# chenchen235/SemStereo

Measured on AMD Instinct MI355X. Metric: stereo pairs/sec, hot segment (gwc+concat volumes, 3-D hourglass stack, soft-argmax), 1024x1024 maxdisp=128, higher is better.
Workload: dtype f32; 1 GPU; BASELINE.json configs[1]: 1024x1024, maxdisp=128, batch=1/GPU x 1 GPU(s); features [B,128,H/4,W/4]+[B,256,H/8,W/8] -> disparity; input_sets_rotated=3, execution=steps round-robin on 6 HIP streams (PairPipeline); bit-identical to one stream, conv_engine=f16x3, hip_graph=False

## Files before the change

include/semstereo_hip.h:

```cpp
#ifndef SEMSTEREO_HIP_H
#define SEMSTEREO_HIP_H

#ifdef __cplusplus
extern "C" {
#endif

typedef void* ss_stream_t;

enum ss_status {
    SS_OK = 0,
    SS_ERR_INVALID = -1,
    SS_ERR_UNSUPPORTED = -2,
    SS_ERR_LAUNCH = -3
};

int ss_abi_version(void);
int ss_reload_tuning(void);
const char* ss_status_string(int status);
const char* ss_last_hip_error(void);


int ss_groupwise_correlation_fwd(const float* fea1, const float* fea2, float* out,
                                 int B, int C, int H, int W, int groups, int normalize,
                                 ss_stream_t stream);
// ... 120 lines not shown
int ss_conv3d_bf16s_cl_fwd(const float* in, const void* wsplit, const float* scale, const float* shift, float* out,
                           int B, int Cin, int D, int H, int W, int Cout, int relu, int nterms, ss_stream_t stream);
int ss_conv3d_head_bf16s_cl_fwd(const float* in, const void* wsplit, const float* scale, const float* shift,
                                float* out, int B, int Cin, int D, int H, int W, int relu, int nterms,
                                ss_stream_t stream);
int ss_pack_classifier_head_weights(const float* w2, void* out, ss_stream_t stream);
int ss_conv3d_classifier_fused_fwd(const float* in, const void* wsplit, const float* scale, const float* shift,
                                   const void* head_w, float* patches, float* out, int B, int Cin, int D, int H, int W,
                                   int nterms, ss_stream_t stream);
int ss_regression_topk_patched_fwd(const float* patches, const float* samples, float* out, int B, int nd, int H, int W, int k,
                                   ss_stream_t stream);
int ss_conv3d_pointwise_bf16s_fwd(const float* in, const void* wsplit, const float* scale, const float* shift,
                                  float* out, int B, int Cin, int Cout, long long npos, int relu, int nterms,
                                  ss_stream_t stream);
int ss_pack_pointwise_weights_bf16s(const float* w, void* wsplit, int Cout, int Cin, ss_stream_t stream);

int ss_deconv3d_fwd(const float* in, const float* wpack, const float* scale, const float* shift,
                    const float* skip, const float* skip_wpack, const float* skip_scale, const float* skip_shift,
                    float* out, int B, int Cin, int D, int H, int W, int Cout, int Cs, int relu,
                    ss_stream_t stream);
int ss_deconv3d_bf16s_fwd(const float* in, const void* wsplit, const float* shift, const float* skip,
                          const void* skip_wsplit, float* out, int B, int Cin, int D, int H, int W, int Cout,
                          int Cs, int relu, int nterms, ss_stream_t stream);
int ss_pack_deconv3d_weights_bf16s(const float* wpack, void* wsplit, int Cin, int Cout, int ntaps, ss_stream_t stream);
int ss_pack_deconv3d_weights_f16s(const float* wpack, void* wsplit, int Cin, int Cout, ss_stream_t stream);
int ss_pack_conv3d_weights(const float* w, float* wpack, int Cout, int Cin, int k, int transposed,
                           ss_stream_t stream);
int ss_conv3d_wgrad_fwd(const float* grad_out, const float* in, float* grad_w, int B, int Cin, int D, int H, int W,
                        int Cout, int stride, ss_stream_t stream);
int ss_conv3d_wgrad_bf16s_fwd(const float* grad_out, const float* in, float* grad_w, float* workspace, int B, int Cin, int D, int H,
// ... 94 lines not shown
```

semstereo_amd/_lib.py:

```python
import ctypes
import os

import torch

_HERE = os.path.dirname(os.path.abspath(__file__))
LIB_PATH = os.path.join(_HERE, "csrc", "libsemstereo_hip.so")
ABI_VERSION = 20

_P = ctypes.c_void_p
_I = ctypes.c_int

_SIGNATURES = {
    "ss_groupwise_correlation_fwd": [_P, _P, _P, _I, _I, _I, _I, _I, _I, _P],
    "ss_gwc_volume_fwd": [_P, _P, _P, _I, _I, _I, _I, _I, _I, _I, _I, _P],
    "ss_gwc_patch_gate_fwd": [_P, _P, _P, _P, _P, _I, _I, _I, _I, _I, _I, _I, _I, _P],
    "ss_gwc_volume_bwd": [_P, _P, _P, _P, _P, _I, _I, _I, _I, _I, _I, _I, _P],
    "ss_concat_volume_fwd": [_P, _P, _P, _I, _I, _I, _I, _I, _I, _I, _P],
    "ss_concat_volume_bwd": [_P, _P, _P, _I, _I, _I, _I, _I, _I, _I, _P],
    "ss_warp_sampled_fwd": [_P, _P, _P, _P, _P, _I, _I, _I, _I, _I, _P],
    "ss_warp_sampled_bwd": [_P, _P, _P, _P, _P, _P, _P, _I, _I, _I, _I, _I, _P],
    "ss_concat_sampled_fwd": [_P, _P, _P, _P, _P, _I, _I, _I, _I, _I, _P],
    "ss_concat_sampled_bwd": [_P, _P, _P, _P, _P, _P, _P, _P, _I, _I, _I, _I, _I, _I, _P],
    "ss_concat_sampled_presplit_fwd": [_P, _P, _P, _P, _P, _I, _I, _I, _I, _I, _P],
    "ss_conv3d_presplit_fwd": [_P, _P, _P, _P, _P, _P, _P, _P, _I, _I, _I, _I, _I, _I, _I, _P],
# ... 27 lines not shown
    "ss_conv2d_bf16s_cat_fwd": [_P, _P, _P, _P, _P, _P, _P, _P, _I, _I, _I, _I, _I, _I, _I, _I, _P],
    "ss_deconv2d_bf16s_fwd": [_P, _P, _P, _P, _P, _I, _I, _I, _I, _I, _I, _I, _P],
    "ss_deconv2d_bf16s_pair_fwd": [_P, _P, _P, _P, _P, _P, _I, _I, _I, _I, _I, _I, _I, _P],
    "ss_pack_deconv2d_weights_f16s": [_P, _P, _I, _I, _P],
    "ss_pack_conv2d_weights_f16s": [_P, _P, _I, _I, _P],
    "ss_conv3d_head_bf16s_fwd": [_P, _P, _P, _P, _P, _I, _I, _I, _I, _I, _I, _I, _P],
    "ss_conv3d_head_bf16s_cl_fwd": [_P, _P, _P, _P, _P, _I, _I, _I, _I, _I, _I, _I, _P],
    "ss_conv3d_bf16s_cl_fwd": [_P, _P, _P, _P, _P, _I, _I, _I, _I, _I, _I, _I, _I, _P],
    "ss_pack_classifier_head_weights": [_P, _P, _P],
    "ss_conv3d_classifier_fused_fwd": [_P, _P, _P, _P, _P, _P, _P, _I, _I, _I, _I, _I, _I, _P],
    "ss_regression_topk_patched_fwd": [_P, _P, _P, _I, _I, _I, _I, _I, _P],
    "ss_pack_conv3d_head_weights_bf16s": [_P, _P, _I, _P],
    "ss_pack_conv3d_head_weights_f16s": [_P, _P, _I, _P],
    "ss_conv3d_pointwise_bf16s_fwd": [_P, _P, _P, _P, _P, _I, _I, _I, ctypes.c_longlong, _I, _I, _P],
    "ss_pack_pointwise_weights_bf16s": [_P, _P, _I, _I, _P],
    "ss_deconv3d_fwd": [_P, _P, _P, _P, _P, _P, _P, _P, _P, _I, _I, _I, _I, _I, _I, _I, _I, _P],
    "ss_pack_deconv3d_weights_f16s": [_P, _P, _I, _I, _P],
    "ss_deconv3d_bf16s_fwd": [_P, _P, _P, _P, _P, _P, _I, _I, _I, _I, _I, _I, _I, _I, _I, _P],
    "ss_pack_deconv3d_weights_bf16s": [_P, _P, _I, _I, _I, _P],
    "ss_pack_conv3d_weights": [_P, _P, _I, _I, _I, _I, _P],
    "ss_conv3d_wgrad_fwd": [_P, _P, _P, _I, _I, _I, _I, _I, _I, _I, _P],
    "ss_conv3d_wgrad_bf16s_fwd": [_P, _P, _P, _P, _I, _I, _I, _I, _I, _I, _I, _P],
    "ss_depthwise_patch_fwd": [_P, _P, _P, _P, _I, _I, _I, _I, _I, _P],
    "ss_window_attention_fwd": [_P, _P, _P, _P, _P, _P, _I, _I, _I, _I, _I, _I, _I, _I, _I, _P],
    "ss_window_attention_core_fwd": [_P, _P, _P, _I, _I, _I, _I, _I, _I, _I, _I, _I, _P],
    "ss_tool_copy_fwd": [_P, _P, ctypes.c_longlong, _P],
    "ss_upsample_softmax_regression_bwd": [_P, _P, _P, _P, _P, _P, _I, _I, _I, _I, _I, _P],
    "ss_sample_strength_bwd": [_P, _P, _P, _P, _P, _P, _P, _P, _P, _P, _P, _P, _I, _I, _I, _I, _P],
    "ss_sample_strength_bwd_ws": [_P, _P, _P, _P, _P, _P, _P, _P, _P, _P, _P, _P, _P, _I, _I, _I, _I, _P],
    "ss_topk_candidates_bwd": [_P, _P, _P, _P, _P, _P, _P, _I, _I, _I, _I, _I, _I, _P],
# ... 94 lines not shown
```

semstereo_amd/csrc/conv3d_head.hip:

```cpp
#include <algorithm>

#include "common.h"
#include "split_f16.h"

namespace {

using f32x16 = __attribute__((ext_vector_type(16))) float;
using bf16x8 = __attribute__((ext_vector_type(8))) short;
using bf16x2_t = __attribute__((ext_vector_type(2))) __bf16;
using f32x2_t = __attribute__((ext_vector_type(2))) float;

constexpr int TWO = 30;

__device__ __forceinline__ unsigned cvt_pk_bf16(float x0, float x1) {
    const f32x2_t v = {x0, x1};
    return __builtin_bit_cast(unsigned, __builtin_convertvector(v, bf16x2_t));
}
__device__ __forceinline__ void split3_pk(float x0, float x1, unsigned& h, unsigned& m, unsigned& l) {
    h = cvt_pk_bf16(x0, x1);
    const float r0 = x0 - __uint_as_float(h << 16), r1 = x1 - __uint_as_float(h & 0xffff0000u);
    m = cvt_pk_bf16(r0, r1);
    const float s0 = r0 - __uint_as_float(m << 16), s1 = r1 - __uint_as_float(m & 0xffff0000u);
    l = cvt_pk_bf16(s0, s1);
}
// ... 244 lines not shown
                           : launch_head_tile<KSV, F16X3>(in, wsplit, scale, shift, out, B, D, H, W, relu, st);
    SS_HEAD(1)
    SS_HEAD(2)
    SS_HEAD(4)
#undef SS_HEAD
    return SS_ERR_UNSUPPORTED;
}

namespace {

template <int KS, int NTERMS>
__global__ __launch_bounds__(256, 2) void pointwise_bf16s(const float* __restrict__ in, const uint4* __restrict__ wsplit,
                                                           const float* __restrict__ scale, const float* __restrict__ shift,
                                                           float* __restrict__ out, int Cout, long long npos,
                                                           int tiles_per_wave, int relu) {
    constexpr int NC = (NTERMS == 6) ? 3 : 2;
    constexpr int Cin = KS * 16;
    const int tid = threadIdx.x, lane = tid & 63, wave = tid >> 6;
    const int l31 = lane & 31, half = lane >> 5;
    const int mt = blockIdx.y * 4 + wave;
    const int b = blockIdx.z;
    if (mt * 32 >= Cout) return;
    bf16x8 a[KS][NC];
#pragma unroll
    for (int ks = 0; ks < KS; ++ks)
#pragma unroll
        for (int c = 0; c < NC; ++c)
            a[ks][c] = __builtin_bit_cast(bf16x8, wsplit[(((size_t)mt * KS + ks) * 3 + c) * 64 + half * 32 + l31]);

    const __amdgpu_buffer_rsrc_t ires = __builtin_amdgcn_make_buffer_rsrc(
        const_cast<float*>(in + (size_t)b * Cin * npos), 0, (int)min((long long)Cin * npos * 4, 0x7fffffffLL), 0x00020000);
    const int chan_b = (int)(npos * 4);
    const __amdgpu_buffer_rsrc_t ores = __builtin_amdgcn_make_buffer_rsrc(
        out + (size_t)b * Cout * npos, 0, (int)min((long long)Cout * npos * 4, 0x7fffffffLL), 0x00020000);
    __shared__ float aff[4][64];
    if (lane < 32) {
        const int co = min(mt * 32 + lane, Cout - 1);
        aff[wave][lane] = scale ? scale[co] : 1.0f;
        aff[wave][32 + lane] = shift ? shift[co] : 0.0f;
    }
    const float floor_v = relu ? 0.f : -__builtin_inff();
    const long long t0 = (long long)blockIdx.x * tiles_per_wave;
    float x[KS][8];
    auto lane_offset = [&](long long tile) {
        const long long p = tile * 32 + l31;
        return (p < npos) ? (unsigned)((8LL * half * npos + p) * 4) : 0x80000000u;
    };
    auto load_step = [&](unsigned off, int ks) {
#pragma unroll
        for (int j = 0; j < 8; ++j)
            x[ks][j] = __builtin_bit_cast(float, __builtin_amdgcn_raw_buffer_load_b32(ires, (int)off, (ks * 16 + j) * chan_b, 0));
    };
    {
        const unsigned off0 = lane_offset(t0);
#pragma unroll
        for (int ks = 0; ks < KS; ++ks) load_step(off0, ks);
    }
#pragma unroll 1
    for (int it = 0; it < tiles_per_wave; ++it) {
        const long long tile = t0 + it;
        if (tile * 32 >= npos) break;
        const unsigned offn = (it + 1 < tiles_per_wave) ? lane_offset(tile + 1) : 0x80000000u;
        f32x16 acc;
#pragma unroll
        for (int q = 0; q < 16; ++q) acc[q] = 0.f;
#pragma unroll
        for (int ks = 0; ks < KS; ++ks) {
            unsigned bh[4], bm[4], bl[4];
#pragma unroll
            for (int j = 0; j < 4; ++j) split3_pk(x[ks][2 * j], x[ks][2 * j + 1], bh[j], bm[j], bl[j]);
            load_step(offn, ks);
            const bf16x8 h8 = __builtin_bit_cast(bf16x8, make_uint4(bh[0], bh[1], bh[2], bh[3]));
            const bf16x8 m8 = __builtin_bit_cast(bf16x8, make_uint4(bm[0], bm[1], bm[2], bm[3]));
            if (NTERMS == 6) {
                const bf16x8 l8 = __builtin_bit_cast(bf16x8, make_uint4(bl[0], bl[1], bl[2], bl[3]));
                acc = __builtin_amdgcn_mfma_f32_32x32x16_bf16(a[ks][1], m8, acc, 0, 0, 0);
                acc = __builtin_amdgcn_mfma_f32_32x32x16_bf16(a[ks][0], l8, acc, 0, 0, 0);
                acc = __builtin_amdgcn_mfma_f32_32x32x16_bf16(a[ks][NC - 1], h8, acc, 0, 0, 0);
            }
            acc = __builtin_amdgcn_mfma_f32_32x32x16_bf16(a[ks][0], m8, acc, 0, 0, 0);
            acc = __builtin_amdgcn_mfma_f32_32x32x16_bf16(a[ks][1], h8, acc, 0, 0, 0);
            acc = __builtin_amdgcn_mfma_f32_32x32x16_bf16(a[ks][0], h8, acc, 0, 0, 0);
        }
        const long long p = tile * 32 + l31;
        const unsigned vo = (p < npos) ? (unsigned)((4LL * half * npos + p) * 4) : 0x80000000u;
#pragma unroll
        for (int r = 0; r < 16; ++r) {
            const int cl = (r & 3) + 8 * (r >> 2);
            const float v = fmaxf(ss::add_rn(ss::mul_rn(acc[r], aff[wave][cl + 4 * half]), aff[wave][32 + cl + 4 * half]), floor_v);
            __builtin_amdgcn_raw_buffer_store_b32(__builtin_bit_cast(unsigned, v), ores,
                                                  (int)((mt * 32 + cl + 4 * half < Cout) ? vo : 0x80000000u), (mt * 32 + cl) * chan_b, 0);
        }
    }
}

__global__ void pack_pointwise_weights_kernel(const float* __restrict__ w, unsigned short* __restrict__ wsplit, int Cout,
                                              int Cin, int total) {
    const int i = blockIdx.x * blockDim.x + threadIdx.x;
    if (i >= total) return;
    const int j = i % 8;
    int r = i / 8;
    const int row = r % 32; r /= 32;
    const int hk = r % 2; r /= 2;
    const int term = r % 3; r /= 3;
    const int KS = Cin / 16;
    const int ks = r % KS;
    const int mt = r / KS;
    const int co = mt * 32 + row, c = ks * 16 + 8 * hk + j;
    const float x = (co < Cout) ? w[(size_t)co * Cin + c] : 0.f;
    unsigned h, m, l;
    split3_pk(x, 0.f, h, m, l);
    wsplit[i] = (unsigned short)((term == 0 ? h : (term == 1 ? m : l)) & 0xffffu);
}

template <int KS, int NTERMS>
int launch_pointwise(const float* in, const void* wsplit, const float* scale, const float* shift, float* out, int B,
                     int Cout, long long npos, int relu, hipStream_t st) {
    const long long ntiles = (npos + 31) / 32;
    const int mgroups = ss::ceil_div(ss::ceil_div(Cout, 32), 4);
    int tpw = 8;
    while (tpw > 1 && ((ntiles + tpw - 1) / tpw) * mgroups * B < 1024) tpw >>= 1;
    const long long gx = (ntiles + tpw - 1) / tpw;
    if (gx > 0x7fffffffLL || B > 65535 || mgroups > 65535) return SS_ERR_UNSUPPORTED;
    hipLaunchKernelGGL((pointwise_bf16s<KS, NTERMS>), dim3((unsigned)gx, mgroups, B), dim3(256), 0, st, in,
                       reinterpret_cast<const uint4*>(wsplit), scale, shift, out, Cout, npos, tpw, relu);
    return ss::check_launch();
}

}

extern "C" int ss_pack_pointwise_weights_bf16s(const float* w, void* wsplit, int Cout, int Cin, ss_stream_t stream) {
    SS_REQUIRE(w && wsplit && Cout > 0 && Cin > 0 && Cin % 16 == 0);
    const int total = ss::ceil_div(Cout, 32) * (Cin / 16) * 3 * 2 * 32 * 8;
    hipLaunchKernelGGL(pack_pointwise_weights_kernel, dim3(ss::ceil_div(total, 256)), dim3(256), 0, ss::as_stream(stream), w,
                       reinterpret_cast<unsigned short*>(wsplit), Cout, Cin, total);
    return ss::check_launch();
}

extern "C" int ss_conv3d_pointwise_bf16s_fwd(const float* in, const void* wsplit, const float* scale, const float* shift,
                                             float* out, int B, int Cin, int Cout, long long npos, int relu, int nterms,
                                             ss_stream_t stream) {
    SS_REQUIRE(in && wsplit && out);
    SS_REQUIRE(B > 0 && Cin > 0 && Cout > 0 && npos > 0 && (nterms == 3 || nterms == 6));
    SS_REQUIRE((reinterpret_cast<uintptr_t>(wsplit) & 15) == 0);
    if ((long long)Cin * npos * 4 >= 0x7fffffffLL) return SS_ERR_UNSUPPORTED;
    if ((long long)Cout * npos * 4 >= 0x7fffffffLL) return SS_ERR_UNSUPPORTED;
    hipStream_t st = ss::as_stream(stream);
#define SS_PW(KSV)                                                                                                    \
    if (Cin == 16 * KSV)                                                                                              \
        return nterms == 6 ? launch_pointwise<KSV, 6>(in, wsplit, scale, shift, out, B, Cout, npos, relu, st)         \
                           : launch_pointwise<KSV, 3>(in, wsplit, scale, shift, out, B, Cout, npos, relu, st);
    SS_PW(2)
    SS_PW(4)
    SS_PW(8)
#undef SS_PW
    return SS_ERR_UNSUPPORTED;
}

extern "C" int ss_conv3d_head_bf16s_cl_fwd(const float* in, const void* wsplit, const float* scale, const float* shift,
                                           float* out, int B, int Cin, int D, int H, int W, int relu, int nterms,
                                           ss_stream_t stream) {
    SS_REQUIRE(in && wsplit && out);
    SS_REQUIRE(B > 0 && Cin > 0 && D > 0 && H > 0 && W > 0 && (nterms == 3 || nterms == 6 || nterms == F16X3));
    SS_REQUIRE(((reinterpret_cast<uintptr_t>(wsplit) | reinterpret_cast<uintptr_t>(in)) & 15) == 0);
    if ((long long)Cin * D * H * W * 4 >= 0x7fffffffLL) return SS_ERR_UNSUPPORTED;
    hipStream_t st = ss::as_stream(stream);
// ... 7 lines not shown
```

semstereo_amd/csrc/stem_left.hip:

```cpp
#include <algorithm>

#include "common.h"

namespace {

constexpr int TH = 8, TW = 32, COG = 4;

template <int ND>
__global__ __launch_bounds__(256) void stem_left_kernel(const float* __restrict__ q, const float* __restrict__ att,
                                                         float* __restrict__ out, int Cout, int H, int W) {
    __shared__ float atile[ND][TH + 2][TW + 2];
    const int tid = threadIdx.x, tx = tid & 31, ty = tid >> 5;
    const int w0 = blockIdx.x * TW, h0 = blockIdx.y * TH;
    const int ngroups = Cout / COG;
    const int b = blockIdx.z / ngroups, co0 = (blockIdx.z % ngroups) * COG;
    const size_t plane = (size_t)H * W;
    const float* ab = att + (size_t)b * ND * plane;
    for (int e = tid; e < ND * (TH + 2) * (TW + 2); e += 256) {
        const int x = e % (TW + 2);
        int r = e / (TW + 2);
        const int y = r % (TH + 2), j = r / (TH + 2);
        const int gh = h0 + y - 1, gw = w0 + x - 1;
        atile[j][y][x] = ((unsigned)gh < (unsigned)H && (unsigned)gw < (unsigned)W) ? ab[(size_t)j * plane + (size_t)gh * W + gw] : 0.f;
    }
// ... 55 lines not shown
        hipLaunchKernelGGL(stem_left_kernel<24>, grid, dim3(256), 0, st, q, att, out, Cout, H, W);
    else if (nd == 32)
        hipLaunchKernelGGL(stem_left_kernel<32>, grid, dim3(256), 0, st, q, att, out, Cout, H, W);
    else if (nd == 6)
        hipLaunchKernelGGL(stem_left_kernel<6>, grid, dim3(256), 0, st, q, att, out, Cout, H, W);
    else
        return SS_ERR_UNSUPPORTED;
    return ss::check_launch();
}

namespace {

using f32x16 = __attribute__((ext_vector_type(16))) float;
using bf16x8 = __attribute__((ext_vector_type(8))) short;
using bf16x2_t = __attribute__((ext_vector_type(2))) __bf16;
using f32x2_t = __attribute__((ext_vector_type(2))) float;

__device__ __forceinline__ unsigned cvt_pk_bf16(float x0, float x1) {
    const f32x2_t v = {x0, x1};
    return __builtin_bit_cast(unsigned, __builtin_convertvector(v, bf16x2_t));
}
__device__ __forceinline__ void split3_pk(float x0, float x1, unsigned& h, unsigned& m, unsigned& l) {
    h = cvt_pk_bf16(x0, x1);
    const float r0 = x0 - __uint_as_float(h << 16), r1 = x1 - __uint_as_float(h & 0xffff0000u);
    m = cvt_pk_bf16(r0, r1);
    const float s0 = r0 - __uint_as_float(m << 16), s1 = r1 - __uint_as_float(m & 0xffff0000u);
    l = cvt_pk_bf16(s0, s1);
}

constexpr int FTH = 4, FTW = 32;
constexpr int HH = FTH + 2, HW = FTW + 2;
constexpr int NPOSH = HH * HW;
constexpr int NNT = (NPOSH + 31) / 32;
constexpr int QCOLS = NNT * 32;

template <int ND, int NTERMS>
__global__ __launch_bounds__(256, 2) void stem_left_fused(const float* __restrict__ left, const uint4* __restrict__ wsplit,
                                                           const float* __restrict__ att, float* __restrict__ out,
                                                           int Cout, int H, int W) {
    constexpr int NC = (NTERMS == 6) ? 3 : 2, KS = 2, C = 32;
    extern __shared__ __attribute__((aligned(16))) float smem[];
    float (*atile)[HH][HW] = reinterpret_cast<float (*)[HH][HW]>(smem) + 1;
    float (*qtile)[QCOLS] = reinterpret_cast<float (*)[QCOLS]>(smem + (ND + 2) * HH * HW);
    const int tid = threadIdx.x, lane = tid & 63, wave = tid >> 6;
    const int l31 = lane & 31, half = lane >> 5;
    const int w0 = blockIdx.x * FTW, h0 = blockIdx.y * FTH, b = blockIdx.z;
    const size_t plane = (size_t)H * W;

    {
        const __amdgpu_buffer_rsrc_t ares = __builtin_amdgcn_make_buffer_rsrc(
            const_cast<float*>(att + (size_t)b * ND * plane), 0, (int)min((long long)ND * (long long)plane * 4, 0x7fffffffLL), 0x00020000);
        constexpr int NE = (ND * NPOSH + 255) / 256;
        float av[NE];
#pragma unroll
        for (int k = 0; k < NE; ++k) {
// ... 9 lines not shown
#pragma unroll
        for (int k = 0; k < NE; ++k) {
            const int e = tid + 256 * k;
            if (e < ND * NPOSH) (&atile[0][0][0])[e] = av[k];
        }
        if (tid < NPOSH) {
            (&atile[-1][0][0])[tid] = 0.f;
            (&atile[ND][0][0])[tid] = 0.f;
        }
    }

    const __amdgpu_buffer_rsrc_t lres = __builtin_amdgcn_make_buffer_rsrc(
        const_cast<float*>(left + (size_t)b * C * plane), 0, (int)min((long long)C * (long long)plane * 4, 0x7fffffffLL), 0x00020000);
    const int chan_b = (int)(plane * 4);
    bf16x8 bfrag[2][KS][NC];
#pragma unroll
    for (int t = 0; t < 2; ++t) {
        const int nt = wave + 4 * t;
        const int p = nt * 32 + l31;
        const int py = p / HW, px = p % HW;
        const int gh = h0 + py - 1, gw = w0 + px - 1;
        const bool ok = nt < NNT && p < NPOSH && (unsigned)gh < (unsigned)H && (unsigned)gw < (unsigned)W;
        const unsigned off = ok ? (unsigned)((8LL * half * plane + (size_t)gh * W + gw) * 4) : 0x80000000u;
#pragma unroll
        for (int ks = 0; ks < KS; ++ks) {
            float x[8];
#pragma unroll
            for (int j = 0; j < 8; ++j)
                x[j] = __builtin_bit_cast(float, __builtin_amdgcn_raw_buffer_load_b32(lres, (int)off, (ks * 16 + j) * chan_b, 0));
            unsigned bh[4], bm[4], bl[4];
// ... 7 lines not shown

    const int jh = tid >> 7, pos = tid & 127, ty = pos >> 5, tx = pos & 31;
    constexpr int NJ = ND / 2;
    static_assert(ND % 2 == 0, "the candidates split over two thread halves");
    const int h = h0 + ty, w = w0 + tx;
    const bool inside = h < H && w < W;
    const int npairs = Cout / 2;
    for (int g = 0; g < npairs; ++g) {
        bf16x8 a[2][KS][NC];
#pragma unroll
        for (int m = 0; m < 2; ++m)
#pragma unroll
            for (int ks = 0; ks < KS; ++ks)
#pragma unroll
                for (int c = 0; c < NC; ++c)
                    a[m][ks][c] = __builtin_bit_cast(bf16x8, wsplit[((((size_t)(g * 2 + m) * KS + ks) * 3 + c) * 2 + half) * 32 + l31]);
        __syncthreads();
#pragma unroll
        for (int t = 0; t < 2; ++t) {
            const int nt = wave + 4 * t;
            if (nt >= NNT) continue;
#pragma unroll
            for (int m = 0; m < 2; ++m) {
                f32x16 acc;
#pragma unroll
                for (int r = 0; r < 16; ++r) acc[r] = 0.f;
#pragma unroll
                for (int ks = 0; ks < KS; ++ks) {
                    if (NTERMS == 6) {
                        acc = __builtin_amdgcn_mfma_f32_32x32x16_bf16(a[m][ks][1], bfrag[t][ks][1], acc, 0, 0, 0);
                        acc = __builtin_amdgcn_mfma_f32_32x32x16_bf16(a[m][ks][0], bfrag[t][ks][NC - 1], acc, 0, 0, 0);
                        acc = __builtin_amdgcn_mfma_f32_32x32x16_bf16(a[m][ks][NC - 1], bfrag[t][ks][0], acc, 0, 0, 0);
                    }
                    acc = __builtin_amdgcn_mfma_f32_32x32x16_bf16(a[m][ks][0], bfrag[t][ks][1], acc, 0, 0, 0);
                    acc = __builtin_amdgcn_mfma_f32_32x32x16_bf16(a[m][ks][1], bfrag[t][ks][0], acc, 0, 0, 0);
                    acc = __builtin_amdgcn_mfma_f32_32x32x16_bf16(a[m][ks][0], bfrag[t][ks][0], acc, 0, 0, 0);
                }
#pragma unroll
                for (int r = 0; r < 16; ++r)
                    qtile[m * 32 + (r & 3) + 8 * (r >> 2) + 4 * half][nt * 32 + l31] = acc[r];
            }
        }
        __syncthreads();
        f32x2_t o[NJ];
#pragma unroll
        for (int j = 0; j < NJ; ++j) o[j] = f32x2_t{0.f, 0.f};
        const int j0 = jh * NJ;
#pragma unroll
        for (int s = 0; s < 9; ++s) {
            const int kh = s / 3, kw = s % 3;
            const int hp = (ty + kh) * HW + tx + kw;
            float av[NJ + 2];
#pragma unroll
            for (int j = -1; j <= NJ; ++j) av[1 + j] = atile[j0 + j][ty + kh][tx + kw];
#pragma unroll
// ... 8 lines not shown
            float* ob = out + (((size_t)b * Cout + 2 * g) * ND + j0) * plane + (size_t)h * W + w;
#pragma unroll
            for (int j = 0; j < NJ; ++j) {
                ob[(size_t)j * plane] = o[j][0];
                ob[((size_t)ND + j) * plane] = o[j][1];
            }
        }
    }
}

template <int ND>
int launch_fused(const float* left, const void* wsplit, const float* att, float* out, int B, int Cout, int H, int W,
                 int nterms, hipStream_t st) {
    const size_t lds = ((size_t)(ND + 2) * HH * HW + 64 * QCOLS) * sizeof(float);
    dim3 grid(ss::ceil_div(W, FTW), ss::ceil_div(H, FTH), B);
    if (nterms == 6) {
        auto kern = stem_left_fused<ND, 6>;
        if (lds > 64 * 1024) {
            if (ss::ensure_dynamic_lds(reinterpret_cast<const void*>(kern), (int)lds) != SS_OK) return SS_ERR_LAUNCH;
        }
        hipLaunchKernelGGL(kern, grid, dim3(256), lds, st, left, reinterpret_cast<const uint4*>(wsplit), att, out, Cout, H, W);
    } else {
        auto kern = stem_left_fused<ND, 3>;
        if (lds > 64 * 1024) {
            if (ss::ensure_dynamic_lds(reinterpret_cast<const void*>(kern), (int)lds) != SS_OK) return SS_ERR_LAUNCH;
        }
        hipLaunchKernelGGL(kern, grid, dim3(256), lds, st, left, reinterpret_cast<const uint4*>(wsplit), att, out, Cout, H, W);
    }
    return ss::check_launch();
}

}

extern "C" int ss_stem_left_fused_fwd(const float* left, const void* wsplit, const float* att, float* out, int B, int C,
                                      int Cout, int nd, int H, int W, int nterms, ss_stream_t stream) {
    SS_REQUIRE(left && wsplit && att && out);
    SS_REQUIRE(B > 0 && C > 0 && Cout > 0 && nd > 0 && H > 0 && W > 0 && (nterms == 3 || nterms == 6));
    SS_REQUIRE((reinterpret_cast<uintptr_t>(wsplit) & 15) == 0);
    if (C != 32 || Cout % 2 != 0 || B > 65535) return SS_ERR_UNSUPPORTED;
    if ((long long)C * H * W * 4 >= 0x7fffffffLL || (long long)nd * H * W * 4 >= 0x7fffffffLL) return SS_ERR_UNSUPPORTED;
    hipStream_t st = ss::as_stream(stream);
    if (nd == 24) return launch_fused<24>(left, wsplit, att, out, B, Cout, H, W, nterms, st);
    if (nd == 32) return launch_fused<32>(left, wsplit, att, out, B, Cout, H, W, nterms, st);
    if (nd == 6) return launch_fused<6>(left, wsplit, att, out, B, Cout, H, W, nterms, st);
    return SS_ERR_UNSUPPORTED;
}
```

semstereo_amd/engine.py:

```python
import os
import weakref

import torch
import torch.nn as nn

from . import _lib, ops
from ._lib import call, ptr

PATH_COUNTS = {"hip": 0, "torch": 0}


def _inference(module, *tensors):
    if module.training:
        return False
    if torch.is_grad_enabled():
        if any(t is not None and t.requires_grad for t in tensors):
            return False
        if any(p.requires_grad for p in module.parameters()):
            return False
        if module.__dict__.get("_is_replica", False):
            for m in module.modules():
                if any(p is not None and p.requires_grad for p in getattr(m, "_former_parameters", {}).values()):
                    return False
    return True
# ... 466 lines not shown
             int(relu), int(nterms))
    return out


def pack_pointwise_weight_bf16s(w):
    w = w.detach().float().reshape(w.shape[0], w.shape[1]).contiguous()
    _lib.require_device(w)
    Cout, Cin = w.shape
    assert Cin % 16 == 0
    out = torch.empty(((Cout + 31) // 32) * (Cin // 16) * 3 * 2 * 32 * 8, dtype=torch.int16, device=w.device)
    with torch.cuda.device(w.device):
        call("ss_pack_pointwise_weights_bf16s", ptr(w), ptr(out), Cout, Cin)
    return out


def conv3d_pointwise_bf16s_hip(x, wsplit, Cout, scale, shift, relu, nterms):
    x = x if x.is_contiguous() else x.contiguous()
    dev = _lib.require_device(x, scale, shift)
    B, Cin = x.shape[0], x.shape[1]
    out = torch.empty((B, Cout) + tuple(x.shape[2:]), dtype=x.dtype, device=x.device)
    with torch.cuda.device(dev):
        call("ss_conv3d_pointwise_bf16s_fwd", ptr(x), ptr(wsplit), ptr(scale), ptr(shift), ptr(out), B, Cin, Cout,
             x[0, 0].numel(), int(relu), int(nterms))
    return out


def _convbn_params(owner, key, conv, bn):
    srcs = [conv.weight] + ([bn.weight, bn.bias, bn.running_mean, bn.running_var] if bn is not None else [])

    def build():
# ... 55 lines not shown
    assert conv.in_channels == 2 * C and _conv_geometry(conv) == (3, 1)
    srcs = [conv.weight] + ([bn.weight, bn.bias, bn.running_mean, bn.running_var] if bn is not None else [])

    def build():
        sc, sh = fold_bn(bn) if bn is not None else (None, None)
        w = conv.weight.detach().float()
        wl = w[:, :C].reshape(Cout, C, 27)
        wq = wl.permute(2, 0, 1).reshape(27 * Cout, C)
        wf = torch.zeros(Cout // 2, 64, C, dtype=w.dtype, device=w.device)
        wf[:, :54] = wl.reshape(Cout // 2, 2, C, 27).permute(0, 3, 1, 2).reshape(Cout // 2, 54, C)
        return (pack_pointwise_weight_bf16s(wq), pack_pointwise_weight_bf16s(wf.reshape(Cout // 2 * 64, C)),
                pack_conv_weight_bf16s(w[:, C:].contiguous(), _tiled_nterms()), sc, sh)
    return _cache(stem).get("bc/halves/" + CONV_ENGINE, srcs, build)


def stem_broadcast_half(stem, left, att):
    assert stem.is_3d and not stem.deconv and CONV_ENGINE != "f32" and _inference(stem, left, att)
    C, Cout = left.shape[1], stem.conv.out_channels
    nterms = _aux_nterms()
    wq, wf, _, _, _ = _stem_halves_params(stem, C)
    PATH_COUNTS["hip"] += 1
    if C == 32 and Cout % 2 == 0 and STEM_LEFT_FUSED:
        return ops.stem_left_fused(left, wf, att, Cout, nterms)
    q = conv3d_pointwise_bf16s_hip(left, wq, 27 * Cout, None, None, False, nterms)
    return ops.stem_left(q, att)


def stem_volume_half(stem, right_vol, partial, gate=None):
    assert stem.is_3d and not stem.deconv and CONV_ENGINE != "f32" and _inference(stem, right_vol, partial, gate)
    nterms = _tiled_nterms()
    _, _, wr, scale, shift = _stem_halves_params(stem, right_vol.shape[1])
    g = None if gate is None else gate.contiguous()
    return conv3d_bf16s_hip(right_vol, wr, stem.conv.out_channels, scale, shift, bool(stem.relu), nterms, None, g, partial=partial)


STEM_PRESPLIT = os.environ.get("SS_STEM_PRESPLIT", "0") != "0"

# ... 48 lines not shown
    if g is not None:
        assert g.shape == (B, Cout, H, W)
    PATH_COUNTS["hip"] += 1
    with torch.cuda.device(dev):
        call("ss_conv3d_gather_fwd", ptr(right), ptr(samples), ptr(att), ptr(wr), ptr(partial), ptr(scale), ptr(shift), ptr(g),
             ptr(out), B, C, nd, H, W, Cout, int(bool(stem.relu)), _tiled_nterms())
    return out


def stem_of_broadcast_and_volume(stem, left, att, right_vol, gate=None):
    return stem_volume_half(stem, right_vol, stem_broadcast_half(stem, left, att), gate)

ATTENTION_FORM = os.environ.get("SS_ATTENTION", "split")

SWITCHES = ("CONV_ENGINE", "DECONV_F16", "DECONV_MIN_WORKGROUPS", "DECONV_BF16S", "CLASSIFIER_CL", "CLASSIFIER_FUSED", "CLASSIFIER_FOLD", "TRAIN_HIP", "SSR_TRAIN_HIP", "LOSS_HIP", "METRICS_HIP", "ATTENTION_FORM",
            "STEM_LEFT_FUSED", "STEM_PRESPLIT", "STEM_GATHER", "STEM_INPLACE", "HEAD_F16", "CONV2D_HIP", "DECODER_HIP")
```

semstereo_amd/modules.py:

```python
import torch
import torch.nn as nn
import torch.nn.functional as F

from . import _lib, ops
from . import deferred as dfr
from . import engine as E
from . import train as T
from . import train_ssr as TS
from ._lib import call, ptr
from .engine import (PATH_COUNTS, _cache, _conv_geometry, _inference, _is_plain_3x3, _ParamCache, _ReplicaCache,
                     classifier_cl_hip, classifier_fused_applies, classifier_fused_hip, pack_classifier_head_weight, conv2d_bf16s_hip, conv3d_bf16s_hip, conv3d_head_bf16s_hip, conv3d_hip,
                     conv3d_pointwise_bf16s_hip, deconv3d_bf16s_hip, deconv3d_hip, fold_bn, pack_conv2d_weight_bf16s,
                     pack_conv_weight, pack_conv_weight_bf16s, pack_deconv_weight_bf16s, pack_head_weight_bf16s,
                     pack_pointwise_weight_bf16s, run_conv2d, run_conv2d_pair, run_convbn, stem_broadcast_half, stem_of_broadcast_and_volume,
                     stem_gather_applies, stem_gather_half, stem_presplit_applies, stem_volume_half, stem_volume_half_presplit, _aux_nterms, _deconv_nterms,
                     _head_nterms, _tiled_nterms)
from .train_layers import (_conv_k3_forward, _deconv_k3_forward, conv3d_train, conv3d_wgrad_hip, deconv3d_train)


class _ConvBN3d(nn.Sequential):

    def forward(self, x):
        x = dfr.real(x)
        if _inference(self, x):
# ... 135 lines not shown
    def _params(self):
        srcs = [self.qkv_3d.weight, self.qkv_3d.bias, self.final1x1.weight, self.final1x1.bias]

        def build():
            C = self.dim_3d
            return (self.qkv_3d.weight.detach().float().t().contiguous(),
                    self.qkv_3d.bias.detach().float().contiguous(),
                    self.final1x1.weight.detach().float().reshape(C, C).t().contiguous(),
                    self.final1x1.bias.detach().float().contiguous())
        return _cache(self).get("attn", srcs, build)

    def _params_split(self):
        srcs = [self.qkv_3d.weight, self.qkv_3d.bias, self.final1x1.weight, self.final1x1.bias]

        bf = E.CONV_ENGINE != "f32" and self.dim_3d in (32, 64, 128)

        def build():
            C = self.dim_3d
            pack = pack_pointwise_weight_bf16s if bf else pack_conv_weight
            return (pack(self.qkv_3d.weight.detach().float().reshape(3 * C, C, 1, 1, 1)),
                    self.qkv_3d.bias.detach().float().contiguous(),
                    pack(self.final1x1.weight.detach().float()),
                    self.final1x1.bias.detach().float().contiguous())
        return _cache(self).get("attn_split/" + ("bf16s" if bf else "f32"), srcs, build) + (bf,)

    def hip_supported(self):
        bd, bh, bw = self.block
        return self.dim_3d == 128 and self.num_heads == 16 and bd * bh * bw in (64, 96)

    def forward(self, x):
        x = dfr.real(x)
        if _inference(self, x) and self.hip_supported():
            PATH_COUNTS["hip"] += 1
            x = x if x.is_contiguous() else x.contiguous()
            dev = _lib.require_device(x)
            B, C, D, H, W = x.shape
            assert C == self.dim_3d and D % self.block[0] == 0
            if E.ATTENTION_FORM == "split":
                wq, bq, wo, bo, bf = self._params_split()
                nterms = _aux_nterms()
                if bf:
                    qkv = conv3d_pointwise_bf16s_hip(x, wq, 3 * C, None, bq, False, nterms)
                else:
                    qkv = conv3d_hip(x, wq, None, bq, 1, 1, False)
                y = torch.empty_like(x)
                with torch.cuda.device(dev):
                    call("ss_window_attention_core_fwd", ptr(qkv), ptr(bq), ptr(y), B, C, D, H, W, self.num_heads,
                         self.block[0], self.block[1], self.block[2])
                if bf:
                    return conv3d_pointwise_bf16s_hip(y, wo, C, None, bo, False, nterms)
                return conv3d_hip(y, wo, None, bo, 1, 1, False)
            wq, bq, wo, bo = self._params()
            out = torch.empty_like(x)
            with torch.cuda.device(dev):
                call("ss_window_attention_fwd", ptr(x), ptr(wq), ptr(bq), ptr(wo), ptr(bo), ptr(out),
# ... 608 lines not shown
```

Measured before the change: 617.3 pairs/s.

## Add scaled f16 split-precision path for pointwise convs and fused left stem

Adds an f16x3 variant of the pointwise 3D conv kernel and the fused left-stem kernel. Weights are packed into two f16 terms with per-row power-of-two scaling, and inputs are scaled per tile. This needs three f16 MFMAs per k-step, where the bf16 split path needed three or six, and it cuts the weight/input split terms from three to two. Both paths are enabled by default when the conv engine is f16x3. In exchange it adds a wave-wide max reduction and a workgroup sync in the stem for input scaling, and it carries a risk of accuracy differences from f16 range and scaling.

```diff
diff --git a/include/semstereo_hip.h b/include/semstereo_hip.h
--- a/include/semstereo_hip.h
+++ b/include/semstereo_hip.h
@@ -158,6 +158,7 @@
                                   float* out, int B, int Cin, int Cout, long long npos, int relu, int nterms,
                                   ss_stream_t stream);
 int ss_pack_pointwise_weights_bf16s(const float* w, void* wsplit, int Cout, int Cin, ss_stream_t stream);
+int ss_pack_pointwise_weights_f16s(const float* w, void* wsplit, int Cout, int Cin, ss_stream_t stream);
 
 int ss_deconv3d_fwd(const float* in, const float* wpack, const float* scale, const float* shift,
                     const float* skip, const float* skip_wpack, const float* skip_scale, const float* skip_shift,
diff --git a/semstereo_amd/_lib.py b/semstereo_amd/_lib.py
--- a/semstereo_amd/_lib.py
+++ b/semstereo_amd/_lib.py
@@ -65,6 +65,7 @@
     "ss_pack_conv3d_head_weights_f16s": [_P, _P, _I, _P],
     "ss_conv3d_pointwise_bf16s_fwd": [_P, _P, _P, _P, _P, _I, _I, _I, ctypes.c_longlong, _I, _I, _P],
     "ss_pack_pointwise_weights_bf16s": [_P, _P, _I, _I, _P],
+    "ss_pack_pointwise_weights_f16s": [_P, _P, _I, _I, _P],
     "ss_deconv3d_fwd": [_P, _P, _P, _P, _P, _P, _P, _P, _P, _I, _I, _I, _I, _I, _I, _I, _I, _P],
     "ss_pack_deconv3d_weights_f16s": [_P, _P, _I, _I, _P],
     "ss_deconv3d_bf16s_fwd": [_P, _P, _P, _P, _P, _P, _I, _I, _I, _I, _I, _I, _I, _I, _I, _P],
diff --git a/semstereo_amd/csrc/conv3d_head.hip b/semstereo_amd/csrc/conv3d_head.hip
--- a/semstereo_amd/csrc/conv3d_head.hip
+++ b/semstereo_amd/csrc/conv3d_head.hip
@@ -282,6 +282,7 @@
                                                            const float* __restrict__ scale, const float* __restrict__ shift,
                                                            float* __restrict__ out, int Cout, long long npos,
                                                            int tiles_per_wave, int relu) {
+    constexpr bool F16 = (NTERMS == F16X3);
     constexpr int NC = (NTERMS == 6) ? 3 : 2;
     constexpr int Cin = KS * 16;
     const int tid = threadIdx.x, lane = tid & 63, wave = tid >> 6;
@@ -294,7 +295,8 @@
     for (int ks = 0; ks < KS; ++ks)
 #pragma unroll
         for (int c = 0; c < NC; ++c)
-            a[ks][c] = __builtin_bit_cast(bf16x8, wsplit[(((size_t)mt * KS + ks) * 3 + c) * 64 + half * 32 + l31]);
+            a[ks][c] = __builtin_bit_cast(bf16x8, wsplit[(((size_t)mt * KS + ks) * (F16 ? 2 : 3) + c) * 64 + half * 32 + l31]);
+    const float* w_unscale = reinterpret_cast<const float*>(wsplit + (size_t)((Cout + 31) / 32) * KS * 2 * 64);
 
     const __amdgpu_buffer_rsrc_t ires = __builtin_amdgcn_make_buffer_rsrc(
         const_cast<float*>(in + (size_t)b * Cin * npos), 0, (int)min((long long)Cin * npos * 4, 0x7fffffffLL), 0x00020000);
@@ -304,7 +306,8 @@
     __shared__ float aff[4][64];
     if (lane < 32) {
         const int co = min(mt * 32 + lane, Cout - 1);
-        aff[wave][lane] = scale ? scale[co] : 1.0f;
+        const float sc = scale ? scale[co] : 1.0f;
+        aff[wave][lane] = F16 ? sc * w_unscale[mt * 32 + lane] : sc;
         aff[wave][32 + lane] = shift ? shift[co] : 0.0f;
     }
     const float floor_v = relu ? 0.f : -__builtin_inff();
@@ -332,6 +335,29 @@
         f32x16 acc;
 #pragma unroll
         for (int q = 0; q < 16; ++q) acc[q] = 0.f;
+        float tile_unscale = 1.0f;
+        if constexpr (F16) {
+            float m = 0.f;
+#pragma unroll
+            for (int ks = 0; ks < KS; ++ks)
+#pragma unroll
+                for (int j = 0; j < 8; ++j) m = fmaxf(m, fabsf(x[ks][j]));
+            const int e = max((int)(wave_max_bits(__float_as_uint(m)) >> 23), E_MIN);
+            const float in_scale = __uint_as_float((unsigned)(127 + E_ONE - e) << 23);
+            tile_unscale = __uint_as_float((unsigned)(127 - E_ONE + e) << 23);
+#pragma unroll
+            for (int ks = 0; ks < KS; ++ks) {
+                unsigned bh[4], bl[4];
+#pragma unroll
+                for (int j = 0; j < 4; ++j) split2_pk_f16(x[ks][2 * j] * in_scale, x[ks][2 * j + 1] * in_scale, bh[j], bl[j]);
+                load_step(offn, ks);
+                const f16x8 h8 = __builtin_bit_cast(f16x8, make_uint4(bh[0], bh[1], bh[2], bh[3]));
+                const f16x8 l8 = __builtin_bit_cast(f16x8, make_uint4(bl[0], bl[1], bl[2], bl[3]));
+                acc = __builtin_amdgcn_mfma_f32_32x32x16_f16(__builtin_bit_cast(f16x8, a[ks][0]), l8, acc, 0, 0, 0);
+                acc = __builtin_amdgcn_mfma_f32_32x32x16_f16(__builtin_bit_cast(f16x8, a[ks][1]), h8, acc, 0, 0, 0);
+                acc = __builtin_amdgcn_mfma_f32_32x32x16_f16(__builtin_bit_cast(f16x8, a[ks][0]), h8, acc, 0, 0, 0);
+            }
+        } else
 #pragma unroll
         for (int ks = 0; ks < KS; ++ks) {
             unsigned bh[4], bm[4], bl[4];
@@ -355,7 +381,8 @@
 #pragma unroll
         for (int r = 0; r < 16; ++r) {
             const int cl = (r & 3) + 8 * (r >> 2);
-            const float v = fmaxf(ss::add_rn(ss::mul_rn(acc[r], aff[wave][cl + 4 * half]), aff[wave][32 + cl + 4 * half]), floor_v);
+            const float av = F16 ? acc[r] * tile_unscale : acc[r];
+            const float v = fmaxf(ss::add_rn(ss::mul_rn(av, aff[wave][cl + 4 * half]), aff[wave][32 + cl + 4 * half]), floor_v);
             __builtin_amdgcn_raw_buffer_store_b32(__builtin_bit_cast(unsigned, v), ores,
                                                   (int)((mt * 32 + cl + 4 * half < Cout) ? vo : 0x80000000u), (mt * 32 + cl) * chan_b, 0);
         }
@@ -381,6 +408,31 @@
     wsplit[i] = (unsigned short)((term == 0 ? h : (term == 1 ? m : l)) & 0xffffu);
 }
 
+__global__ void pack_pointwise_weights_f16s_kernel(const float* __restrict__ w, unsigned short* __restrict__ wsplit, int Cout,
+                                                   int Cin, int total) {
+    const int i = blockIdx.x * blockDim.x + threadIdx.x;
+    if (i >= total) return;
+    const int j = i % 8;
+    int r = i / 8;
+    const int row = r % 32; r /= 32;
+    const int hk = r % 2; r /= 2;
+    const int term = r % 2; r /= 2;
+    const int KS = Cin / 16;
+    const int ks = r % KS;
+    const int mt = r / KS;
+    const int co = mt * 32 + row, c = ks * 16 + 8 * hk + j;
+    float m = 0.f;
+    if (co < Cout)
+        for (int k = 0; k < Cin; ++k) m = fmaxf(m, fabsf(w[(size_t)co * Cin + k]));
+    const int e = max((int)(__float_as_uint(m) >> 23), E_MIN);
+    const float unscale = __uint_as_float((unsigned)(127 - E_ONE + e) << 23);
+    if (term == 0 && hk == 0 && ks == 0 && j == 0) reinterpret_cast<float*>(wsplit + total)[co] = unscale;
+    const float x = (co < Cout) ? w[(size_t)co * Cin + c] / unscale : 0.f;
+    const _Float16 h = (_Float16)x;
+    const _Float16 l = (_Float16)(x - (float)h);
+    wsplit[i] = __builtin_bit_cast(unsigned short, term == 0 ? h : l);
+}
+
 template <int KS, int NTERMS>
 int launch_pointwise(const float* in, const void* wsplit, const float* scale, const float* shift, float* out, int B,
                      int Cout, long long npos, int relu, hipStream_t st) {
@@ -405,11 +457,20 @@
     return ss::check_launch();
 }
 
+extern "C" int ss_pack_pointwise_weights_f16s(const float* w, void* wsplit, int Cout, int Cin, ss_stream_t stream) {
+    SS_REQUIRE(w && wsplit && Cout > 0 && Cin > 0 && Cin % 16 == 0);
+    SS_REQUIRE((reinterpret_cast<uintptr_t>(wsplit) & 15) == 0);
+    const int total = ss::ceil_div(Cout, 32) * (Cin / 16) * 2 * 2 * 32 * 8;
+    hipLaunchKernelGGL(pack_pointwise_weights_f16s_kernel, dim3(ss::ceil_div(total, 256)), dim3(256), 0, ss::as_stream(stream), w,
+                       reinterpret_cast<unsigned short*>(wsplit), Cout, Cin, total);
+    return ss::check_launch();
+}
+
 extern "C" int ss_conv3d_pointwise_bf16s_fwd(const float* in, const void* wsplit, const float* scale, const float* shift,
                                              float* out, int B, int Cin, int Cout, long long npos, int relu, int nterms,
                                              ss_stream_t stream) {
     SS_REQUIRE(in && wsplit && out);
-    SS_REQUIRE(B > 0 && Cin > 0 && Cout > 0 && npos > 0 && (nterms == 3 || nterms == 6));
+    SS_REQUIRE(B > 0 && Cin > 0 && Cout > 0 && npos > 0 && (nterms == 3 || nterms == 6 || nterms == F16X3));
     SS_REQUIRE((reinterpret_cast<uintptr_t>(wsplit) & 15) == 0);
     if ((long long)Cin * npos * 4 >= 0x7fffffffLL) return SS_ERR_UNSUPPORTED;
     if ((long long)Cout * npos * 4 >= 0x7fffffffLL) return SS_ERR_UNSUPPORTED;
@@ -417,7 +478,8 @@
 #define SS_PW(KSV)                                                                                                    \
     if (Cin == 16 * KSV)                                                                                              \
         return nterms == 6 ? launch_pointwise<KSV, 6>(in, wsplit, scale, shift, out, B, Cout, npos, relu, st)         \
-                           : launch_pointwise<KSV, 3>(in, wsplit, scale, shift, out, B, Cout, npos, relu, st);
+             : nterms == 3 ? launch_pointwise<KSV, 3>(in, wsplit, scale, shift, out, B, Cout, npos, relu, st)         \
+                           : launch_pointwise<KSV, F16X3>(in, wsplit, scale, shift, out, B, Cout, npos, relu, st);
     SS_PW(2)
     SS_PW(4)
     SS_PW(8)
diff --git a/semstereo_amd/csrc/stem_left.hip b/semstereo_amd/csrc/stem_left.hip
--- a/semstereo_amd/csrc/stem_left.hip
+++ b/semstereo_amd/csrc/stem_left.hip
@@ -1,6 +1,7 @@
 #include <algorithm>
 
 #include "common.h"
+#include "split_f16.h"
 
 namespace {
 
@@ -93,7 +94,6 @@
 using f32x16 = __attribute__((ext_vector_type(16))) float;
 using bf16x8 = __attribute__((ext_vector_type(8))) short;
 using bf16x2_t = __attribute__((ext_vector_type(2))) __bf16;
-using f32x2_t = __attribute__((ext_vector_type(2))) float;
 
 __device__ __forceinline__ unsigned cvt_pk_bf16(float x0, float x1) {
     const f32x2_t v = {x0, x1};
@@ -117,7 +117,9 @@
 __global__ __launch_bounds__(256, 2) void stem_left_fused(const float* __restrict__ left, const uint4* __restrict__ wsplit,
                                                            const float* __restrict__ att, float* __restrict__ out,
                                                            int Cout, int H, int W) {
+    constexpr bool F16 = (NTERMS == F16X3);
     constexpr int NC = (NTERMS == 6) ? 3 : 2, KS = 2, C = 32;
+    __shared__ unsigned wgmax[4];
     extern __shared__ __attribute__((aligned(16))) float smem[];
     float (*atile)[HH][HW] = reinterpret_cast<float (*)[HH][HW]>(smem) + 1;
     float (*qtile)[QCOLS] = reinterpret_cast<float (*)[QCOLS]>(smem + (ND + 2) * HH * HW);
@@ -157,6 +159,43 @@
         const_cast<float*>(left + (size_t)b * C * plane), 0, (int)min((long long)C * (long long)plane * 4, 0x7fffffffLL), 0x00020000);
     const int chan_b = (int)(plane * 4);
     bf16x8 bfrag[2][KS][NC];
+    float x_unscale = 1.0f;
+    if constexpr (F16) {
+        float xs[2][KS][8];
+        float mx = 0.f;
+#pragma unroll
+        for (int t = 0; t < 2; ++t) {
+            const int nt = wave + 4 * t;
+            const int p = nt * 32 + l31;
+            const int py = p / HW, px = p % HW;
+            const int gh = h0 + py - 1, gw = w0 + px - 1;
+            const bool ok = nt < NNT && p < NPOSH && (unsigned)gh < (unsigned)H && (unsigned)gw < (unsigned)W;
+            const unsigned off = ok ? (unsigned)((8LL * half * plane + (size_t)gh * W + gw) * 4) : 0x80000000u;
+#pragma unroll
+            for (int ks = 0; ks < KS; ++ks)
+#pragma unroll
+                for (int j = 0; j < 8; ++j) {
+                    xs[t][ks][j] = __builtin_bit_cast(float, __builtin_amdgcn_raw_buffer_load_b32(lres, (int)off, (ks * 16 + j) * chan_b, 0));
+                    mx = fmaxf(mx, fabsf(xs[t][ks][j]));
+                }
+        }
+        const unsigned wm = wave_max_bits(__float_as_uint(mx));
+        if (lane == 0) wgmax[wave] = wm;
+        __syncthreads();
+        const int e = max((int)(max(max(wgmax[0], wgmax[1]), max(wgmax[2], wgmax[3])) >> 23), E_MIN);
+        const float in_scale = __uint_as_float((unsigned)(127 + E_ONE - e) << 23);
+        x_unscale = __uint_as_float((unsigned)(127 - E_ONE + e) << 23);
+#pragma unroll
+        for (int t = 0; t < 2; ++t)
+#pragma unroll
+            for (int ks = 0; ks < KS; ++ks) {
+                unsigned bh[4], bl[4];
+#pragma unroll
+                for (int j = 0; j < 4; ++j) split2_pk_f16(xs[t][ks][2 * j] * in_scale, xs[t][ks][2 * j + 1] * in_scale, bh[j], bl[j]);
+                bfrag[t][ks][0] = __builtin_bit_cast(bf16x8, make_uint4(bh[0], bh[1], bh[2], bh[3]));
+                bfrag[t][ks][1] = __builtin_bit_cast(bf16x8, make_uint4(bl[0], bl[1], bl[2], bl[3]));
+            }
+    } else
 #pragma unroll
     for (int t = 0; t < 2; ++t) {
         const int nt = wave + 4 * t;
@@ -194,7 +233,18 @@
             for (int ks = 0; ks < KS; ++ks)
 #pragma unroll
                 for (int c = 0; c < NC; ++c)
-                    a[m][ks][c] = __builtin_bit_cast(bf16x8, wsplit[((((size_t)(g * 2 + m) * KS + ks) * 3 + c) * 2 + half) * 32 + l31]);
+                    a[m][ks][c] = __builtin_bit_cast(bf16x8, wsplit[((((size_t)(g * 2 + m) * KS + ks) * (F16 ? 2 : 3) + c) * 2 + half) * 32 + l31]);
+        float4 un[2][4];
+        if constexpr (F16) {
+            const float4* w_unscale = reinterpret_cast<const float4*>(wsplit + (size_t)Cout * KS * 2 * 64);
+#pragma unroll
+            for (int m = 0; m < 2; ++m)
+#pragma unroll
+                for (int q = 0; q < 4; ++q) {
+                    const float4 u = w_unscale[(g * 2 + m) * 8 + 2 * q + half];
+                    un[m][q] = make_float4(u.x * x_unscale, u.y * x_unscale, u.z * x_unscale, u.w * x_unscale);
+                }
+        }
         __syncthreads();
 #pragma unroll
         for (int t = 0; t < 2; ++t) {
@@ -207,6 +257,14 @@
                 for (int r = 0; r < 16; ++r) acc[r] = 0.f;
 #pragma unroll
                 for (int ks = 0; ks < KS; ++ks) {
+                    if constexpr (F16) {
+                        const f16x8 ah = __builtin_bit_cast(f16x8, a[m][ks][0]), al = __builtin_bit_cast(f16x8, a[m][ks][1]);
+                        const f16x8 xh = __builtin_bit_cast(f16x8, bfrag[t][ks][0]), xl = __builtin_bit_cast(f16x8, bfrag[t][ks][1]);
+                        acc = __builtin_amdgcn_mfma_f32_32x32x16_f16(ah, xl, acc, 0, 0, 0);
+                        acc = __builtin_amdgcn_mfma_f32_32x32x16_f16(al, xh, acc, 0, 0, 0);
+                        acc = __builtin_amdgcn_mfma_f32_32x32x16_f16(ah, xh, acc, 0, 0, 0);
+                        continue;
+                    }
                     if (NTERMS == 6) {
                         acc = __builtin_amdgcn_mfma_f32_32x32x16_bf16(a[m][ks][1], bfrag[t][ks][1], acc, 0, 0, 0);
                         acc = __builtin_amdgcn_mfma_f32_32x32x16_bf16(a[m][ks][0], bfrag[t][ks][NC - 1], acc, 0, 0, 0);
@@ -217,8 +275,14 @@
                     acc = __builtin_amdgcn_mfma_f32_32x32x16_bf16(a[m][ks][0], bfrag[t][ks][0], acc, 0, 0, 0);
                 }
 #pragma unroll
-                for (int r = 0; r < 16; ++r)
-                    qtile[m * 32 + (r & 3) + 8 * (r >> 2) + 4 * half][nt * 32 + l31] = acc[r];
+                for (int r = 0; r < 16; ++r) {
+                    float v = acc[r];
+                    if constexpr (F16) {
+                        const float4 u = un[m][r >> 2];
+                        v *= (r & 3) == 0 ? u.x : (r & 3) == 1 ? u.y : (r & 3) == 2 ? u.z : u.w;
+                    }
+                    qtile[m * 32 + (r & 3) + 8 * (r >> 2) + 4 * half][nt * 32 + l31] = v;
+                }
             }
         }
         __syncthreads();
@@ -257,7 +321,13 @@
                  int nterms, hipStream_t st) {
     const size_t lds = ((size_t)(ND + 2) * HH * HW + 64 * QCOLS) * sizeof(float);
     dim3 grid(ss::ceil_div(W, FTW), ss::ceil_div(H, FTH), B);
-    if (nterms == 6) {
+    if (nterms == F16X3) {
+        auto kern = stem_left_fused<ND, F16X3>;
+        if (lds > 64 * 1024) {
+            if (ss::ensure_dynamic_lds(reinterpret_cast<const void*>(kern), (int)lds) != SS_OK) return SS_ERR_LAUNCH;
+        }
+        hipLaunchKernelGGL(kern, grid, dim3(256), lds, st, left, reinterpret_cast<const uint4*>(wsplit), att, out, Cout, H, W);
+    } else if (nterms == 6) {
         auto kern = stem_left_fused<ND, 6>;
         if (lds > 64 * 1024) {
             if (ss::ensure_dynamic_lds(reinterpret_cast<const void*>(kern), (int)lds) != SS_OK) return SS_ERR_LAUNCH;
@@ -278,7 +348,7 @@
 extern "C" int ss_stem_left_fused_fwd(const float* left, const void* wsplit, const float* att, float* out, int B, int C,
                                       int Cout, int nd, int H, int W, int nterms, ss_stream_t stream) {
     SS_REQUIRE(left && wsplit && att && out);
-    SS_REQUIRE(B > 0 && C > 0 && Cout > 0 && nd > 0 && H > 0 && W > 0 && (nterms == 3 || nterms == 6));
+    SS_REQUIRE(B > 0 && C > 0 && Cout > 0 && nd > 0 && H > 0 && W > 0 && (nterms == 3 || nterms == 6 || nterms == F16X3));
     SS_REQUIRE((reinterpret_cast<uintptr_t>(wsplit) & 15) == 0);
     if (C != 32 || Cout % 2 != 0 || B > 65535) return SS_ERR_UNSUPPORTED;
     if ((long long)C * H * W * 4 >= 0x7fffffffLL || (long long)nd * H * W * 4 >= 0x7fffffffLL) return SS_ERR_UNSUPPORTED;
diff --git a/semstereo_amd/engine.py b/semstereo_amd/engine.py
--- a/semstereo_amd/engine.py
+++ b/semstereo_amd/engine.py
@@ -504,6 +504,34 @@
     return out
 
 
+def pack_pointwise_weight_f16s(w):
+    w = w.detach().float().reshape(w.shape[0], w.shape[1]).contiguous()
+    _lib.require_device(w)
+    Cout, Cin = w.shape
+    assert Cin % 16 == 0
+    mt = (Cout + 31) // 32
+    out = torch.empty(mt * (Cin // 16) * 2 * 2 * 32 * 8 + mt * 32 * 2, dtype=torch.int16, device=w.device)
+    with torch.cuda.device(w.device):
+        call("ss_pack_pointwise_weights_f16s", ptr(w), ptr(out), Cout, Cin)
+    return out
+
+
+POINTWISE_F16 = os.environ.get("SS_POINTWISE_F16", "1") != "0"
+STEM_LEFT_F16 = os.environ.get("SS_STEM_LEFT_F16", "1") != "0"
+
+
+def _pointwise_nterms():
+    return 19 if (CONV_ENGINE == "f16x3" and POINTWISE_F16) else _aux_nterms()
+
+
+def _stem_left_nterms():
+    return 19 if (CONV_ENGINE == "f16x3" and STEM_LEFT_F16) else _aux_nterms()
+
+
+def pack_pointwise_weight(w, nterms):
+    return pack_pointwise_weight_f16s(w) if nterms == 19 else pack_pointwise_weight_bf16s(w)
+
+
 def conv3d_pointwise_bf16s_hip(x, wsplit, Cout, scale, shift, relu, nterms):
     x = x if x.is_contiguous() else x.contiguous()
     dev = _lib.require_device(x, scale, shift)
@@ -589,6 +617,18 @@
     return _cache(stem).get("bc/halves/" + CONV_ENGINE, srcs, build)
 
 
+def _stem_left_f16_params(stem, C):
+    conv = stem.conv
+    Cout = conv.out_channels
+
+    def build():
+        wl = conv.weight.detach().float()[:, :C].reshape(Cout, C, 27)
+        wf = torch.zeros(Cout // 2, 64, C, dtype=wl.dtype, device=wl.device)
+        wf[:, :54] = wl.reshape(Cout // 2, 2, C, 27).permute(0, 3, 1, 2).reshape(Cout // 2, 54, C)
+        return (pack_pointwise_weight_f16s(wf.reshape(Cout // 2 * 64, C)),)
+    return _cache(stem).get("bc/left_f16", [conv.weight], build)[0]
+
+
 def stem_broadcast_half(stem, left, att):
     assert stem.is_3d and not stem.deconv and CONV_ENGINE != "f32" and _inference(stem, left, att)
     C, Cout = left.shape[1], stem.conv.out_channels
@@ -596,6 +636,8 @@
     wq, wf, _, _, _ = _stem_halves_params(stem, C)
     PATH_COUNTS["hip"] += 1
     if C == 32 and Cout % 2 == 0 and STEM_LEFT_FUSED:
+        if _stem_left_nterms() == 19:
+            return ops.stem_left_fused(left, _stem_left_f16_params(stem, C), att, Cout, 19)
         return ops.stem_left_fused(left, wf, att, Cout, nterms)
     q = conv3d_pointwise_bf16s_hip(left, wq, 27 * Cout, None, None, False, nterms)
     return ops.stem_left(q, att)
@@ -674,4 +716,4 @@
 ATTENTION_FORM = os.environ.get("SS_ATTENTION", "split")
 
 SWITCHES = ("CONV_ENGINE", "DECONV_F16", "DECONV_MIN_WORKGROUPS", "DECONV_BF16S", "CLASSIFIER_CL", "CLASSIFIER_FUSED", "CLASSIFIER_FOLD", "TRAIN_HIP", "SSR_TRAIN_HIP", "LOSS_HIP", "METRICS_HIP", "ATTENTION_FORM",
-            "STEM_LEFT_FUSED", "STEM_PRESPLIT", "STEM_GATHER", "STEM_INPLACE", "HEAD_F16", "CONV2D_HIP", "DECODER_HIP")
+            "STEM_LEFT_FUSED", "STEM_LEFT_F16", "POINTWISE_F16", "STEM_PRESPLIT", "STEM_GATHER", "STEM_INPLACE", "HEAD_F16", "CONV2D_HIP", "DECODER_HIP")
diff --git a/semstereo_amd/modules.py b/semstereo_amd/modules.py
--- a/semstereo_amd/modules.py
+++ b/semstereo_amd/modules.py
@@ -173,15 +173,16 @@
         srcs = [self.qkv_3d.weight, self.qkv_3d.bias, self.final1x1.weight, self.final1x1.bias]
 
         bf = E.CONV_ENGINE != "f32" and self.dim_3d in (32, 64, 128)
+        nterms = E._pointwise_nterms() if bf else 0
 
         def build():
             C = self.dim_3d
-            pack = pack_pointwise_weight_bf16s if bf else pack_conv_weight
+            pack = (lambda w: E.pack_pointwise_weight(w, nterms)) if bf else pack_conv_weight
             return (pack(self.qkv_3d.weight.detach().float().reshape(3 * C, C, 1, 1, 1)),
                     self.qkv_3d.bias.detach().float().contiguous(),
                     pack(self.final1x1.weight.detach().float()),
                     self.final1x1.bias.detach().float().contiguous())
-        return _cache(self).get("attn_split/" + ("bf16s" if bf else "f32"), srcs, build) + (bf,)
+        return _cache(self).get("attn_split/" + (("f16s" if nterms == 19 else "bf16s") if bf else "f32"), srcs, build) + (bf, nterms)
 
     def hip_supported(self):
         bd, bh, bw = self.block
@@ -196,8 +197,7 @@
             B, C, D, H, W = x.shape
             assert C == self.dim_3d and D % self.block[0] == 0
             if E.ATTENTION_FORM == "split":
-                wq, bq, wo, bo, bf = self._params_split()
-                nterms = _aux_nterms()
+                wq, bq, wo, bo, bf, nterms = self._params_split()
                 if bf:
                     qkv = conv3d_pointwise_bf16s_hip(x, wq, 3 * C, None, bq, False, nterms)
                 else:
```

After: 621.8 pairs/s, median of 6. About the same (+0.7%).
